# NTT123/vietTTS

Hardware: AMD Instinct MI355X
Metric: audio samples/sec whole-node, HiFi-GAN V1 mel2wave (higher is better)
Workload: dtype bf16; 1 GPU; HiFi-GAN V1 generator, 64 utterances x 1024 mel frames per GPU per step (BASELINE configs[2] shape), bf16; batch_per_gpu=64, frames=1024, parallelism=dp1 utterance-sharded, weights broadcast once, no data-path collective, microbatch=0, streams=0, schedule=engine default: micro-batches of <= 32768 frames on two HIP streams

## Files before the change

viettts_amd/csrc/engine.hip:

```cpp
#include "../../include/vtts_hifigan.h"

#include <hip/hip_runtime.h>

#include <cmath>
#include <cstdarg>
#include <cstdio>
#include <cstring>
#include <string>
#include <vector>

#include "vtts_internal.h"

using namespace vtts;

namespace {

thread_local std::string g_last_error;

}

int vtts::failf(int code, const char* fmt, ...) {
    char buf[512];
    va_list ap;
    va_start(ap, fmt);
// ... 50 lines not shown
    int64_t opt_profile = 0;
    int cur_b0 = 0;
    const int* cur_lens = nullptr;
    int cur_T = 0;
    int64_t opt_tiles = 0;
    int64_t opt_fuse = 2;
    int64_t opt_streams = 0;
    int64_t opt_graph = 1;
    struct GraphEntry {
        const void* mel = nullptr;
        void* wav = nullptr;
        void* ws = nullptr;
        int B = 0, T = 0, seen = 0;
        uint64_t epoch = 0, last_use = 0;
        hipGraph_t graph = nullptr;
        hipGraphExec_t exec = nullptr;
    };
    std::vector<GraphEntry> graphs;
    hipStream_t cap_stream = nullptr;
    uint64_t epoch = 0, use_clock = 0;
    int64_t opt_zigzag = 1;
    unsigned zrev_count = 0;
    int64_t opt_tail = 1;
    int64_t opt_chains = 1;
    hipEvent_t ev_chain[3] = {nullptr, nullptr, nullptr};
    hipStream_t side_streams[3] = {nullptr, nullptr, nullptr};
    hipEvent_t ev_fork = nullptr, ev_join[3] = {nullptr, nullptr, nullptr};
    int prof_C = 0, prof_K = 0;
    std::vector<std::pair<hipEvent_t, hipEvent_t>> prof_events;
    size_t prof_used = 0;
    double prof_flops = 0.0;
    std::string prof_name, prof_name_pair;
};

namespace {

int conv_same_pad_a(int k, int s) {
    const int pad_len = k + s - 2;
    return (s > k - 1) ? (k - 1) : (pad_len + 1) / 2;
}

void pick_dominant_class(vtts_hifigan* h, bool mfma_only) {
    double best_flops = -1.0;
    for (const Layer& l : h->layers) {
        if (&l == &h->layers[h->idx_pre] || l.kind != KIND_CONV || l.cin != l.cout || (mfma_only && !l.has_wp)) continue;
        double fl = 0.0;
// ... 423 lines not shown
    return launch_timed(h, l, 1, B, L, s, "bf16 kernel launch",
                        [&] { return ug ? launch_convt_g_bf16(l.bcls, a, s) : launch_conv_bf16(l.bcls, K, a, s); });
}

BConvArgs resblock_args_bf16(vtts_hifigan* h, const Layer& c1, const void* x, int B, int L, float slope_out, void* y, int acc_add, float div) {
    BConvArgs a;
    memset(&a, 0, sizeof(a));
    a.x = x;
    a.y = y;
    a.B = B;
    a.L = L;
    set_ragged(h, a, L);
    a.x_pitch = c1.cin;
    a.cin_real = c1.cin;
    a.slope_in = 0.1f;
    a.slope_out = slope_out;
    a.acc_add = acc_add;
    a.div = div;
    a.zrev = next_zrev(h);
    return a;
}

int run_pair_bf16(vtts_hifigan* h, const Layer& c1, const void* x, int B, int L, float slope_out, void* y, int acc_add, float div,
                  hipStream_t s, float* tail_wav = nullptr) {
    BConvArgs a = resblock_args_bf16(h, c1, x, B, L, slope_out, y, acc_add, div);
    a.wp = h->blob + c1.off_pw;
    a.bias = reinterpret_cast<const float*>(h->blob + c1.off_pb);
    a.dil = c1.dil;
    a.pad = c1.pad;
    a.tile_pref = (int)h->opt_tiles;
    if (tail_wav) {
        const Layer& post = h->layers[h->idx_post];
        a.tail_wav = tail_wav;
        a.tail_wf = reinterpret_cast<const float*>(h->blob + post.off_w);
        a.tail_bias = reinterpret_cast<const float*>(h->blob + post.off_b);
    }
    return launch_timed(h, c1, 2, B, L, s, "fused pair launch", [&] { return launch_pair_g_bf16(c1.cin, c1.k, a, s); });
}

int run_resblock_bf16(vtts_hifigan* h, const Layer* rb, const void* x, int B, int L, float slope_out, void* y, int acc_add, float div,
                      hipStream_t s) {
    BConvArgs a = resblock_args_bf16(h, rb[0], x, B, L, slope_out, y, acc_add, div);
    a.wp = h->blob + rb[0].off_rw;
    a.bias = reinterpret_cast<const float*>(h->blob + rb[0].off_rb);
    a.dils[0] = rb[0].dil;
    a.dils[1] = rb[2].dil;
    a.dils[2] = rb[4].dil;
    return launch_timed(h, rb[0], 0, B, L, s, "fused ResBlock launch", [&] { return launch_resblock_bf16(rb[0].cin, rb[0].k, a, s); });
}

Route route_bf16(const vtts_hifigan* h, const Layer* rb) {
    if (h->opt_fuse >= 2 && rb[0].has_rb && (h->opt_fuse >= 3 || resblock_bf16_preferred(rb[0].cin, rb[0].k))) return ROUTE_RESBLOCK;
    if (h->opt_fuse >= 1 && rb[0].has_pair && rb[2].has_pair && rb[4].has_pair) return ROUTE_PAIRS;
    return ROUTE_CONVS;
}

bool tail_fused_bf16(const vtts_hifigan* h) {
    if (!h->opt_tail || h->cfg.resblock == 2) return false;
    const Layer* rb = &h->layers[h->idx_res.back()];
    const Layer& post = h->layers[h->idx_post];
    return route_bf16(h, rb) == ROUTE_PAIRS && pair_tail_bf16_supported(rb[0].cin, rb[0].k, post.cin, post.cout, post.k);
}

size_t elem_bytes(const vtts_hifigan* h) { return h->dtype == VTTS_BF16 ? 2 : sizeof(float); }

size_t max_act_elems(const vtts_hifigan* h, int T) {
    size_t best = (size_t)h->cfg.upsample_initial_channel * T;
    long L = T;
    for (int i = 0; i < h->cfg.num_upsamples; ++i) {
        L *= h->cfg.upsample_rates[i];
        size_t e = (size_t)(h->cfg.upsample_initial_channel >> (i + 1)) * L;
        if (e > best) best = e;
    }
    return best;
}

int auto_streams(const vtts_hifigan* h) { return h->opt_streams > 0 ? (int)h->opt_streams : 2; }

int pass_frames(const vtts_hifigan* h) { return (h->dtype == VTTS_F32 && auto_streams(h) >= 2) ? 32768 : 65536; }

int microbatch_frames(const vtts_hifigan* h) { return auto_streams(h) >= 2 ? 32768 : 65536; }

int pick_microbatch(const vtts_hifigan* h, int B, int T) {
    if (h->opt_microbatch > 0) return (int)std::min<int64_t>(h->opt_microbatch, B);
// ... 95 lines not shown
    hipStream_t cs[4];
    int rc = fork_streams(h, nk, s, cs);
    for (int j = 0; j < nk && !rc; ++j) rc = chain(j, cs[j]);
    const int rj = join_streams(h, nk, s);
    return rc ? rc : rj;
}

struct Taps {
    const char* name = nullptr;
    float* out = nullptr;
    bool is(const char* tap, int i = -1) const {
        if (!name) return false;
        return i < 0 ? !strcmp(name, tap) : !strncmp(name, tap, 4) && atoi(name + 4) == i;
    }
};

struct MicroBatch {
    int b0, nb;
    hipStream_t s;
    PassBufs buf;
    bool par;
    float* wav;
    bool tail;
};

int tap_copy(const vtts_hifigan* h, const MicroBatch& m, const void* src, float* dst, size_t n) {
    const hipError_t e = h->dtype == VTTS_BF16 ? launch_bf16_to_f32(src, dst, n, m.s)
                                               : hipMemcpyAsync(dst, src, n * sizeof(float), hipMemcpyDeviceToDevice, m.s);
    if (e != hipSuccess) return failf(VTTS_ERR_HIP, "tap copy failed: %s", hipGetErrorString(e));
    return VTTS_OK;
}

__global__ __launch_bounds__(256) void mrf_mean_k(const float* __restrict__ y0, const float* __restrict__ y1, const float* __restrict__ y2,
                                                  float* __restrict__ out, size_t n, float div) {
    for (size_t i = (size_t)blockIdx.x * 256 + threadIdx.x; i < n; i += (size_t)gridDim.x * 256) {
        float v = y0[i] + y1[i];
        if (y2) v = v + y2[i];
        out[i] = v / div;
    }
}

float* f32(char* p) { return reinterpret_cast<float*>(p); }

int conv_pre_f32(vtts_hifigan* h, const MicroBatch& m, const float* mel, int T) {
    const int nm = h->cfg.num_mels;
    return run_layer(h, h->layers[h->idx_pre], Act{mel, (long)T * nm, 1, nm}, m.nb, T, 1.0f, nullptr, f32(m.buf.S), ACC_STORE, 1.f, 0,
// ... 76 lines not shown
    auto run_chain = [&](int j, hipStream_t cs, auto before_last) -> int {
        const Layer* rb = &h->layers[h->idx_res[i * nk + j]];
        char* tT = m.buf.T[j];
        char* tC = m.buf.C[j];
        const char* cur = m.buf.X;
        const bool last_rb = j == nk - 1;
        const float slope = last_rb ? next_slope : 1.0f;
        const int acc = j > 0 ? 1 : 0;
        const float div = last_rb ? (float)nk : 1.0f;
        int rc;
        if (c.resblock == 2) {
            if ((rc = run_layer_bf16(h, rb[0], cur, C, C, m.nb, L, 0.1f, 1.0f, cur, tC, 0, 1.f, cs))) return rc;
            if ((rc = before_last())) return rc;
            return run_layer_bf16(h, rb[1], tC, C, C, m.nb, L, 0.1f, slope, tC, m.buf.S, acc, div, cs);
        }
        switch (route_bf16(h, rb)) {
            case ROUTE_RESBLOCK:
                if ((rc = before_last())) return rc;
                return run_resblock_bf16(h, rb, cur, m.nb, L, slope, m.buf.S, acc, div, cs);
            case ROUTE_PAIRS:
                if ((rc = run_pair_bf16(h, rb[0], cur, m.nb, L, 1.0f, tT, 0, 1.f, cs))) return rc;
                if ((rc = run_pair_bf16(h, rb[2], tT, m.nb, L, 1.0f, tC, 0, 1.f, cs))) return rc;
                if ((rc = before_last())) return rc;
                return run_pair_bf16(h, rb[4], tC, m.nb, L, slope, m.buf.S, acc, div, cs, last_stage && last_rb && m.tail ? m.wav : nullptr);
            default:
                for (int z = 0; z < 2; ++z) {
                    if ((rc = run_layer_bf16(h, rb[2 * z], cur, C, C, m.nb, L, 0.1f, 0.1f, nullptr, tT, 0, 1.f, cs))) return rc;
                    if ((rc = run_layer_bf16(h, rb[2 * z + 1], tT, C, C, m.nb, L, 1.0f, 1.0f, cur, tC, 0, 1.f, cs))) return rc;
                    cur = tC;
                }
                if ((rc = run_layer_bf16(h, rb[4], cur, C, C, m.nb, L, 0.1f, 0.1f, nullptr, tT, 0, 1.f, cs))) return rc;
                if ((rc = before_last())) return rc;
                return run_layer_bf16(h, rb[5], tT, C, C, m.nb, L, 1.0f, slope, cur, m.buf.S, acc, div, cs);
        }
    };
    if (!m.par) {
        for (int j = 0; j < nk; ++j)
            if (int rc = run_chain(j, m.s, [] { return VTTS_OK; })) return rc;
        return VTTS_OK;
    }
    auto hip_rc = [&](hipError_t e, const char* what) -> int {
        return e == hipSuccess ? VTTS_OK : failf(VTTS_ERR_HIP, "%s failed: %s", what, hipGetErrorString(e));
    };
    return run_chains_parallel(h, nk, m.s, [&](int j, hipStream_t cs) -> int {
        int rc = run_chain(j, cs, [&]() -> int {
            return j > 0 ? hip_rc(hipStreamWaitEvent(cs, h->ev_chain[j - 1], 0), "hipStreamWaitEvent(chain)") : VTTS_OK;
// ... 19 lines not shown
    hipError_t e = launch_conv_post_bf16(a, m.wav, pre_act, m.s);
    if (e != hipSuccess) return failf(VTTS_ERR_HIP, "conv_post launch failed: %s", hipGetErrorString(e));
    return VTTS_OK;
}

struct Engine {
    int (*conv_pre)(vtts_hifigan*, const MicroBatch&, const float* mel, int T);
    int (*upsample)(vtts_hifigan*, const MicroBatch&, int i, int L);
    int (*mrf)(vtts_hifigan*, const MicroBatch&, int i, int L);
    int (*conv_post)(vtts_hifigan*, const MicroBatch&, int L, float* pre_act);
};
constexpr Engine ENGINE_F32{conv_pre_f32, upsample_f32, mrf_f32, conv_post_f32};
constexpr Engine ENGINE_BF16{conv_pre_bf16, upsample_bf16, mrf_bf16, conv_post_bf16};

int run_micro_batch(vtts_hifigan* h, const Engine& e, const MicroBatch& m, const float* mel, int T, const Taps& tap) {
    const vtts_hifigan_cfg& c = h->cfg;
    const Layer& pre = h->layers[h->idx_pre];
    int rc;
    if ((rc = e.conv_pre(h, m, mel + (size_t)m.b0 * T * c.num_mels, T))) return rc;
    if (tap.is("conv_pre") && (rc = tap_copy(h, m, m.buf.S, tap.out + (size_t)m.b0 * pre.cout * T, (size_t)m.nb * pre.cout * T))) return rc;
    long L = T;
    for (int i = 0; i < c.num_upsamples; ++i) {
        const Layer& up = h->layers[h->idx_ups[i]];
        if ((rc = e.upsample(h, m, i, (int)L))) return rc;
        L *= up.stride;
        const size_t CL = (size_t)up.cout * L;
        if (tap.is("ups_", i) && (rc = tap_copy(h, m, m.buf.X, tap.out + (size_t)m.b0 * CL, (size_t)m.nb * CL))) return rc;
        if ((rc = e.mrf(h, m, i, (int)L))) return rc;
        if (tap.is("mrf_", i) && (rc = tap_copy(h, m, m.buf.S, tap.out + (size_t)m.b0 * CL, (size_t)m.nb * CL))) return rc;
    }
    if (m.tail) return VTTS_OK;
    return e.conv_post(h, m, (int)L, tap.is("pre_tanh") ? tap.out + (size_t)m.b0 * h->hop * T : nullptr);
}

int forward_impl(vtts_hifigan* h, const float* mel, int B, int T, float* wav, void* ws, size_t ws_bytes, hipStream_t s0,
                 const Taps& tap) {
    if (!h->blob) return failf(VTTS_ERR_STATE, "forward() before pack()/bind_packed()");
    if (B <= 0 || T <= 0) return failf(VTTS_ERR_INVALID, "B and T must be positive (got B=%d, T=%d)", B, T);
    if (int rc = check_pass_size(h, B, T)) return rc;
    const PassPlan p = plan_pass(h, B, T);
    if (ws_bytes < p.bytes() || !ws) return failf(VTTS_ERR_NOMEM, "workspace too small: %zu < %zu bytes", ws_bytes, p.bytes());
    if ((reinterpret_cast<uintptr_t>(ws) & 255) != 0) return failf(VTTS_ERR_INVALID, "workspace must be 256-B aligned");
    {
        hipError_t e = hipSetDevice(h->device);
        if (e != hipSuccess) return failf(VTTS_ERR_HIP, "hipSetDevice(%d) failed: %s", h->device, hipGetErrorString(e));
    }
    const Engine& e = h->dtype == VTTS_BF16 ? ENGINE_BF16 : ENGINE_F32;
    const bool tail = h->dtype == VTTS_BF16 && !tap.name && tail_fused_bf16(h);
    hipStream_t streams[4];
    int rc = fork_streams(h, p.nstr, s0, streams);
    for (int b0 = 0; b0 < B && !rc; b0 += p.mb) {
        const int si = (b0 / p.mb) % p.nstr;
        const MicroBatch m{b0, std::min(p.mb, B - b0), streams[si], p.buffers(ws, si, h->cfg.num_kernels), p.par, wav + (size_t)b0 * h->hop * T, tail};
        h->cur_b0 = b0;
        rc = run_micro_batch(h, e, m, mel, T, tap);
    }
    const int rj = join_streams(h, p.nstr, s0);
    return rc ? rc : rj;
}

}

VTTS_API int vtts_abi_version(void) { return VTTS_ABI_VERSION; }

VTTS_API const char* vtts_last_error(void) { return g_last_error.c_str(); }

VTTS_API int vtts_hifigan_create(const vtts_hifigan_cfg* cfg, int device, int dtype, vtts_hifigan** out) {
    if (!cfg || !out) return failf(VTTS_ERR_INVALID, "null argument");
    *out = nullptr;
    if (dtype != VTTS_F32 && dtype != VTTS_BF16 && dtype != VTTS_BF16X3) return failf(VTTS_ERR_INVALID, "unknown dtype %d", dtype);
    if (cfg->num_upsamples < 1 || cfg->num_upsamples > VTTS_MAX_UPSAMPLES)
        return failf(VTTS_ERR_INVALID, "num_upsamples %d out of range", cfg->num_upsamples);
    if (cfg->num_kernels < 1 || cfg->num_kernels > VTTS_MAX_KERNELS)
        return failf(VTTS_ERR_INVALID, "num_kernels %d out of range", cfg->num_kernels);
    if (cfg->num_mels < 1 || cfg->upsample_initial_channel < 1)
        return failf(VTTS_ERR_INVALID, "num_mels / upsample_initial_channel must be positive");
// ... 482 lines not shown
    HIP_TRY(hipMalloc(&ybuf.p, n * 2));
    if (route == 1) {
        HIP_TRY(hipMalloc(&tbuf.p, n * 2));
        HIP_TRY(hipMalloc(&cbuf.p, n * 2));
    }
    int rc = VTTS_OK;
    if (launch_f32_to_bf16(x_dev, xbuf.p, n, st) != hipSuccess || launch_f32_to_bf16(y_dev, ybuf.p, n, st) != hipSuccess)
        rc = failf(VTTS_ERR_HIP, "conversion launch failed");
    if (!rc && route == 0) rc = run_resblock_bf16(h, rb, xbuf.p, B, L, slope_out, ybuf.p, acc_add, div, st);
    if (!rc && route == 1) {
        rc = run_pair_bf16(h, rb[0], xbuf.p, B, L, 1.0f, tbuf.p, 0, 1.f, st);
        if (!rc) rc = run_pair_bf16(h, rb[2], tbuf.p, B, L, 1.0f, cbuf.p, 0, 1.f, st);
        if (!rc) rc = run_pair_bf16(h, rb[4], cbuf.p, B, L, slope_out, ybuf.p, acc_add, div, st);
    }
    if (!rc && launch_bf16_to_f32(ybuf.p, y_dev, n, st) != hipSuccess) rc = failf(VTTS_ERR_HIP, "conversion launch failed");
    hipError_t e = hipStreamSynchronize(st);
    if (!rc && e != hipSuccess) rc = failf(VTTS_ERR_HIP, "run_resblock failed: %s", hipGetErrorString(e));
    return rc;
}

VTTS_API int vtts_hifigan_set_option(vtts_hifigan* h, const char* name, int64_t value) {
    if (!h || !name) return failf(VTTS_ERR_INVALID, "null argument");
    {
        static const char* const writable[] = {"kernels", "microbatch", "fuse", "streams", "graph", "zigzag", "chains", "tiles", "tail", "stage"};
        for (const char* w : writable) {
            int64_t cur = 0;
            if (!strcmp(name, w) && vtts_hifigan_get_option(h, name, &cur) == VTTS_OK && cur == value) return VTTS_OK;
        }
    }
    ++h->epoch;
    if (!strcmp(name, "kernels")) {
        if (value != 0 && value != 1) return failf(VTTS_ERR_INVALID, "kernels must be 0 (auto) or 1 (generic)");
        h->opt_kernels = value;
    } else if (!strcmp(name, "microbatch")) {
        if (value < 0) return failf(VTTS_ERR_INVALID, "microbatch must be >= 0");
        h->opt_microbatch = value;
    } else if (!strcmp(name, "fuse")) {
        if (value < 0 || value > 3) return failf(VTTS_ERR_INVALID, "fuse must be 0 (per convolution), 1 (pairs), 2 (bf16: pairs + whole ResBlocks where faster; fp32: pairs at C <= 64) or 3 (... wherever supported)");
        h->opt_fuse = value;
    } else if (!strcmp(name, "streams")) {
        if (value < 0 || value > 4) return failf(VTTS_ERR_INVALID, "streams must be 1..4 (0 = the engine's default)");
        h->opt_streams = value;
    } else if (!strcmp(name, "graph")) {
        if (value != 0 && value != 1) return failf(VTTS_ERR_INVALID, "graph must be 0 (always eager) or 1 (small launches replay a captured hipGraph)");
        h->opt_graph = value;
    } else if (!strcmp(name, "zigzag")) {
        if (value != 0 && value != 1) return failf(VTTS_ERR_INVALID, "zigzag must be 0 or 1");
        h->opt_zigzag = value;
    } else if (!strcmp(name, "chains")) {
        if (value < 0 || value > 2) return failf(VTTS_ERR_INVALID, "chains must be 0 (ResBlocks of a stage one after the other), 1 (side by side on small fp32 launches) or 2 (... on every single-micro-batch launch)");
        h->opt_chains = value;
    } else if (!strcmp(name, "tiles")) {
        if (value < 0 || value > 2) return failf(VTTS_ERR_INVALID, "tiles must be 0 (auto), 1 (wide) or 2 (narrow)");
        h->opt_tiles = value;
    } else if (!strcmp(name, "tail")) {
        if (value != 0 && value != 1) return failf(VTTS_ERR_INVALID, "tail must be 0 or 1");
        h->opt_tail = value;
    } else if (!strcmp(name, "stage")) {
        if (value != 0) return failf(VTTS_ERR_INVALID, "stage must be 0: the whole-stage kernel was removed (it measured slower, profiles/r06_a_stage_kernel_findings.md)");
    } else if (!strcmp(name, "profile")) {
        h->opt_profile = value ? 1 : 0;
    } else if (!strcmp(name, "hop") || !strcmp(name, "pass_frames") || !strcmp(name, "max_frames_per_pass") || !strcmp(name, "graphs_cached") ||
               !strcmp(name, "profile_C") || !strcmp(name, "profile_K")) {
        return failf(VTTS_ERR_INVALID, "option '%s' is read-only", name);
    } else {
        return failf(VTTS_ERR_INVALID, "unknown option '%s'", name);
    }
    return VTTS_OK;
}

VTTS_API int vtts_hifigan_get_option(const vtts_hifigan* h, const char* name, int64_t* value) {
    if (!h || !name || !value) return failf(VTTS_ERR_INVALID, "null argument");
    if (!strcmp(name, "kernels")) *value = h->opt_kernels;
    else if (!strcmp(name, "microbatch")) *value = h->opt_microbatch;
    else if (!strcmp(name, "profile")) *value = h->opt_profile;
    else if (!strcmp(name, "tiles")) *value = h->opt_tiles;
    else if (!strcmp(name, "streams")) *value = h->opt_streams;
    else if (!strcmp(name, "zigzag")) *value = h->opt_zigzag;
    else if (!strcmp(name, "chains")) *value = h->opt_chains;
    else if (!strcmp(name, "graph")) *value = h->opt_graph;
    else if (!strcmp(name, "tail")) *value = h->opt_tail;
    else if (!strcmp(name, "stage")) *value = 0;
    else if (!strcmp(name, "graphs_cached")) {
        *value = 0;
        for (auto& g : h->graphs) *value += g.exec ? 1 : 0;
    }
    else if (!strcmp(name, "fuse")) *value = h->opt_fuse;
    else if (!strcmp(name, "hop")) *value = h->hop;
    else if (!strcmp(name, "max_frames_per_pass")) {
        const size_t per = max_act_elems(h, 1) * elem_bytes(h);
        *value = (int64_t)((((size_t)1 << 31) + per - 1) / per);
    }
    else if (!strcmp(name, "pass_frames")) *value = pass_frames(h);
    else if (!strcmp(name, "profile_C")) *value = h->prof_C;
    else if (!strcmp(name, "profile_K")) *value = h->prof_K;
    else return failf(VTTS_ERR_INVALID, "unknown option '%s'", name);
    return VTTS_OK;
}

VTTS_API int vtts_hifigan_profile_read(vtts_hifigan* h, double* resblock_ms, int64_t* launches, double* resblock_flops,
                                       int reset) {
    if (!h) return failf(VTTS_ERR_INVALID, "null argument");
    double ms = 0.0;
    for (size_t i = 0; i < h->prof_used; ++i) {
// ... 20 lines not shown
```

viettts_amd/csrc/kernels_bf16_rbg.hip:

```cpp
#include <stdio.h>
#include <string.h>

#include <type_traits>
#include <utility>

#include "bf16_common.h"

namespace vtts {

template <class F, int... I>
__device__ __forceinline__ void static_for(std::integer_sequence<int, I...>, F&& f) {
    (f(std::integral_constant<int, I>{}), ...);
}

constexpr int XCD_MAP_MIN_TILES = 192;

template <int C_, int KS_, int N1_, int WM_, int WN_, int PA_, int MINWG_, int XC_ = C_, int BLK_ = 32>
struct GTile {
    static constexpr int C = C_, KS = KS_, N1 = N1_, WM = WM_, WN = WN_, PA = PA_, MINWG = MINWG_, BLK = BLK_;
    static constexpr int XC = XC_, NXC = C / XC;
    static constexpr int MR16 = C / WM / 16, NR16 = N1 / WN / 16, NH = NR16 / 4;
    static constexpr int KS32 = C / 32, KSX32 = XC / 32;
        static constexpr int LA16 = 3, RA16 = LA16 + 1;
    static_assert(BLK == 32 || BLK == 16, "MFMA block shape");
// ... 9 lines not shown
    static constexpr int ROWST = N1 + 2 * H2;
    static constexpr int KSTEPS = C / 16;
    static constexpr int KSX = XC / 16;
    static constexpr int NQT = KS * KSTEPS;
    static constexpr int MB = C / 32;
    static constexpr int RA = PA + 1;
    static constexpr bool UNROLL_ALL = (KSX % RA) != 0;
    static constexpr bool WREG = UNROLL_ALL && NXC == 1 && NQT * MR * 4 <= 96;
    static constexpr int XPT = (ROWSX_MAX * SPR1 + THREADS - 1) / THREADS;
    static constexpr size_t CONV_BYTES = (size_t)KS * C * C * 2;
    static_assert(C % (WM * 32) == 0 && N1 % (WN * 32) == 0, "tile/wave mismatch");
    static_assert(C % XC == 0 && (NXC == 1 || !UNROLL_ALL), "channel chunking");
    static_assert(SPR1 == 4 || SPR1 == 8 || SPR1 == 16, "X row pitch 64..256 B");
    static_assert(SPR2 == 4 || SPR2 == 8 || SPR2 == 16 || SPR2 == 32, "xt row pitch 64..512 B");
    static constexpr bool RAWRES = NXC == 1 && C == 32;
    static constexpr int RAW_BYTES = RAWRES ? tile_rows16(N1) * P1 : 0;
    static __host__ __device__ constexpr int tile_bytes(int dil) {
        const int bx = tile_rows16(N1 + 2 * H2 * dil) * P1, bt = tile_rows16(ROWST) * P2;
        return bx > bt ? bx : bt;
    }
    static constexpr bool TAIL = false;
    static constexpr int TAIL_KS = 7, TAIL_H = 3;
    static constexpr int TAIL_BYTES = 0;
    static int lds_bytes(int dil) { return tile_bytes(dil) + RAW_BYTES; }
    static_assert(tile_rows16(ROWSX_MAX) * P1 + RAW_BYTES <= 80 * 1024 || !RAWRES, "two workgroups per CU");
    static_assert(tile_rows16(ROWSX_MAX) * P1 <= 160 * 1024 && tile_rows16(ROWST) * P2 <= 160 * 1024, "LDS budget");
};

template <class B>
struct GTail : B {
    static constexpr bool TAIL = true;
    static constexpr int TAIL_BYTES = 1024;
    static int lds_bytes(int dil) { return B::tile_bytes(dil) + B::RAW_BYTES + TAIL_BYTES; }
    static_assert(B::RAWRES && B::C == 32 && B::WM == 1, "the tail lives on the C = 32 tile with the LDS-resident residual rows");
    static_assert(B::tile_bytes(B::MAXDIL) + B::RAW_BYTES + TAIL_BYTES <= 80 * 1024, "two workgroups per CU");
};

template <class T>
__global__ __launch_bounds__(T::THREADS, (T::MINWG * T::THREADS + 255) / 256) void resblock_pair_g_bf16_k(BConvArgs a) {
    constexpr int C = T::C, KS = T::KS, N1 = T::N1, WN = T::WN, PA = T::PA, RA = T::RA;
    constexpr int THREADS = T::THREADS, MR = T::MR, NR = T::NR, H2 = T::H2, NT2 = T::NT2;
    constexpr int SPR1 = T::SPR1, P1 = T::P1, SPR2 = T::SPR2, P2 = T::P2, XC = T::XC, NXC = T::NXC, KSX = T::KSX;
    constexpr int KSTEPS = T::KSTEPS, NQT = T::NQT, MB = T::MB, XPT = T::XPT;
    constexpr int BLK = T::BLK;
    constexpr bool B16 = BLK == 16;
    constexpr int MR16 = T::MR16, NR16 = T::NR16, NH = T::NH;
    static_assert(!B16 || (!T::RAWRES && !T::TAIL && !T::WREG && !T::UNROLL_ALL), "16-block tiles are the rolled-loop C >= 64 tiles");

    extern __shared__ __attribute__((aligned(16))) unsigned char lds[];
    unsigned char* xt = lds;
    [[maybe_unused]] unsigned char* const xraw = lds + (T::RAWRES ? T::tile_bytes(a.dil) : 0);

    const int tid = threadIdx.x;
    const int lane = tid & 63;
    const int wave = tid >> 6;
    const int wm = wave / WN;
    const int wn = wave % WN;
    const int l31 = lane & 31;
    const int lh = lane >> 5;
    const int l15 = lane & 15;
    const int lg = lane >> 4;
    const int b = a.zrev ? (int)(gridDim.z - 1 - blockIdx.z) : (int)blockIdx.z;
    const int Lp = a.L;
    const int L = a.lens ? min(max(a.lens[b], 0) * a.len_mul, a.L) : a.L;
    constexpr int TS = T::TAIL ? NT2 - 2 * T::TAIL_H : NT2;
    const bool xmap = (a.L + TS - 1) / TS >= XCD_MAP_MIN_TILES;
    const int nt = (L + TS - 1) / TS, r = (int)((blockIdx.x + b) & 7), lo = (r * nt) >> 3, hi = ((r + 1) * nt) >> 3;
    const int tile = xmap ? lo + (int)(blockIdx.x >> 3) : (int)blockIdx.x;
    if (xmap && tile >= hi) return;
    const int t0 = tile * TS - (T::TAIL ? T::TAIL_H : 0);
    if (t0 + (T::TAIL ? T::TAIL_H : 0) >= L) return;
    const int dil = a.dil;
    const int h1 = H2 * dil;
    const int rowsx = N1 + 2 * h1;
    const unsigned short* __restrict__ xg = static_cast<const unsigned short*>(a.x) + (size_t)b * Lp * C;
    [[maybe_unused]] const int wg_lin = blockIdx.z * gridDim.x + blockIdx.x;
    VTTS_TL_ID(a, wg_lin);
    VTTS_TL(a, wg_lin, 0);

    typedef float f32x4 __attribute__((ext_vector_type(4)));
    f32x16 acc[B16 ? 1 : MR][B16 ? 1 : NR];
    f32x16 bblk[B16 ? 1 : MR];
    f32x4 acc16[B16 ? MR16 : 1][B16 ? NR16 : 1];
    f32x4 bblk16[B16 ? MR16 : 1];
    auto load_bias = [&](const float* __restrict__ bias) {
        typedef float f32x8 __attribute__((ext_vector_type(8)));
        if constexpr (B16) {
#pragma unroll
            for (int mr = 0; mr < MR16; ++mr) bblk16[mr] = *reinterpret_cast<const f32x4*>(bias + wm * (C / T::WM) + mr * 16 + 4 * lg);
            return;
        }
#pragma unroll
        for (int mr = 0; mr < MR; ++mr) {
            const float* __restrict__ bp = bias + wm * (C / T::WM) + mr * 32 + 4 * lh;
// ... 479 lines not shown
        };
        if constexpr (T::RAWRES) {
#pragma unroll
            for (int mr = 0; mr < MR; ++mr)
#pragma unroll
                for (int p = 0; p < 2; ++p)
#pragma unroll
                    for (int nr = 0; nr < NR; ++nr) {
                        const int col = wn * (N1 / WN) + nr * 32 + l31;
                        uint4 r = *reinterpret_cast<const uint4*>(xraw + tile_off<SPR1, BLK>(col, (wm * (C / T::WM) + mr * 32 + 16 * p) / 8 + lh));
                        swap_pair(r.x, r.z);
                        swap_pair(r.y, r.w);
                        const int r0 = 8 * p;
                        acc[mr][nr][r0 + 0] = vadd_raw(bf16_lo(r.x), acc[mr][nr][r0 + 0]); acc[mr][nr][r0 + 1] = vadd_raw(bf16_hi(r.x), acc[mr][nr][r0 + 1]);
                        acc[mr][nr][r0 + 2] = vadd_raw(bf16_lo(r.y), acc[mr][nr][r0 + 2]); acc[mr][nr][r0 + 3] = vadd_raw(bf16_hi(r.y), acc[mr][nr][r0 + 3]);
                        acc[mr][nr][r0 + 4] = vadd_raw(bf16_lo(r.z), acc[mr][nr][r0 + 4]); acc[mr][nr][r0 + 5] = vadd_raw(bf16_hi(r.z), acc[mr][nr][r0 + 5]);
                        acc[mr][nr][r0 + 6] = vadd_raw(bf16_lo(r.w), acc[mr][nr][r0 + 6]); acc[mr][nr][r0 + 7] = vadd_raw(bf16_hi(r.w), acc[mr][nr][r0 + 7]);
                    }
        } else {
            add_rows(xg);
        }
        if (a.acc_add != 0) add_rows(yg);
        VTTS_TL(a, wg_lin, 12);
        if constexpr (B16) {
#pragma unroll
            for (int mr = 0; mr < MR16; ++mr) {
                const int cb = wm * (C / T::WM) + mr * 16;
#pragma unroll
                for (int j = 0; j < NR16 / 2; ++j) {
                    const int row = col16 + 32 * j;
                    const int t = t0 + row;
                    const bool ok = row < NT2 && t >= 0 && t < L;
                    float v[8];
#pragma unroll
                    for (int e = 0; e < 4; ++e) {
                        v[e] = acc16[mr][2 * j][e];
                        v[4 + e] = acc16[mr][2 * j + 1][e];
                    }
                    if (dv != 1.0f) {
#pragma unroll
                        for (int e = 0; e < 8; ++e) v[e] = v[e] * rdv;
                    }
                    if (s_out != 1.0f) {
#pragma unroll
                        for (int e = 0; e < 8; ++e) v[e] = lrelu_f(v[e], s_out);
                    }
                    unsigned p0 = pack_bf16x2(v[0], v[1]), p1 = pack_bf16x2(v[2], v[3]);
                    unsigned q0 = pack_bf16x2(v[4], v[5]), q1 = pack_bf16x2(v[6], v[7]);
                    swap_pair16(p0, q0);
                    swap_pair16(p1, q1);
                    if (ok) *reinterpret_cast<uint4*>(yg + (size_t)t * C + cb + 8 * (lg >> 1)) = make_uint4(p0, p1, q0, q1);
                }
            }
        } else {
#pragma unroll
        for (int mr = 0; mr < MR; ++mr) {
#pragma unroll
            for (int p = 0; p < 2; ++p) {
                const int cb = wm * (C / T::WM) + mr * 32 + 16 * p;
#pragma unroll
                for (int nr = 0; nr < NR; ++nr) {
                    const int row = wn * (N1 / WN) + nr * 32 + l31;
                    const int t = t0 + row;
                    const bool ok = row < NT2 && t >= 0 && t < L;
                    float v[8];
#pragma unroll
                    for (int e = 0; e < 8; ++e) v[e] = acc[mr][nr][8 * p + e];
                    if (dv != 1.0f) {
#pragma unroll
                        for (int e = 0; e < 8; ++e) v[e] = v[e] * rdv;
                    }
                    if (s_out != 1.0f) {
#pragma unroll
                        for (int e = 0; e < 8; ++e) v[e] = lrelu_f(v[e], s_out);
                    }
                    unsigned p0 = pack_bf16x2(v[0], v[1]), p1 = pack_bf16x2(v[2], v[3]);
                    unsigned q0 = pack_bf16x2(v[4], v[5]), q1 = pack_bf16x2(v[6], v[7]);
                    swap_pair(p0, q0);
                    swap_pair(p1, q1);
                    if constexpr (T::TAIL) {
                        const uint4 o = ok ? make_uint4(p0, p1, q0, q1) : make_uint4(0u, 0u, 0u, 0u);
                        if (row < NT2) *reinterpret_cast<uint4*>(xraw + tile_off<SPR1, BLK>(row, (cb >> 3) + lh)) = o;
                    } else {
                        if (ok) *reinterpret_cast<uint4*>(yg + (size_t)t * C + cb + 8 * lh) = make_uint4(p0, p1, q0, q1);
                    }
                }
            }
        }
        }
    }
    if constexpr (T::TAIL) {
        __syncthreads();
        const float* tw = reinterpret_cast<const float*>(lds + T::tile_bytes(dil) + T::RAW_BYTES);
        const float tb = a.tail_bias[0];
        for (int n = tid; n < TS; n += THREADS) {
            const int t = t0 + T::TAIL_H + n;
            if (t >= L) break;
            float accp = 0.f;
#pragma unroll
            for (int j = 0; j < T::TAIL_KS; ++j) {
#pragma unroll
                for (int c = 0; c < SPR1; ++c) {
                    const uint4 v = *reinterpret_cast<const uint4*>(xraw + tile_off<SPR1, BLK>(n + j, c));
                    const float* w = tw + j * C + c * 8;
                    accp = fmaf(w[0], bf16_lo(v.x), accp); accp = fmaf(w[1], bf16_hi(v.x), accp);
                    accp = fmaf(w[2], bf16_lo(v.y), accp); accp = fmaf(w[3], bf16_hi(v.y), accp);
                    accp = fmaf(w[4], bf16_lo(v.z), accp); accp = fmaf(w[5], bf16_hi(v.z), accp);
                    accp = fmaf(w[6], bf16_lo(v.w), accp); accp = fmaf(w[7], bf16_hi(v.w), accp);
                }
            }
            a.tail_wav[(size_t)b * Lp + t] = tanhf(accp + tb);
        }
// ... 19 lines not shown
constexpr int g_mfma_blk(int C, int KS) {
    return C == 256 ? (KS == 3 ? 16 : KS == 7 ? 32 : 16)
         : C == 128 ? (KS == 3 ? 16 : KS == 7 ? 16 : 16)
         : C == 64  ? (KS == 3 ? 32 : KS == 7 ? 16 : 16)
                    : 32;
}
template <int KS> using G128 = GTile<128, KS, KS == 3 ? VTTS_G128K3_N1 : 256, 2, 2, 3, KS == 3 ? VTTS_G128K3_WG : 2, 128, g_mfma_blk(128, KS)>;
template <int KS> using G64 = GTile<64, KS, VTTS_G64_N1, 1, 4, 3, VTTS_G64_WG, 64, g_mfma_blk(64, KS)>;
#ifndef VTTS_G32_PA
#define VTTS_G32_PA 3
#endif
template <int KS> using G32 = GTile<32, KS, VTTS_G32_N1, 1, 4, VTTS_G32_PA, VTTS_G32_WG>;
template <int KS> using G256 = GTile<256, KS, 128, 4, 1, 3, 2, 128, g_mfma_blk(256, KS)>;
template <int KS> using G256S = GTile<256, KS, 64, 4, 1, 3, 2, 128, g_mfma_blk(256, KS)>;
template <int KS> using G128S = GTile<128, KS, 128, 2, 2, 3, 2, 128, g_mfma_blk(128, KS)>;
template <int KS> using G64S = GTile<64, KS, 256, 1, 4, 3, 2, 64, g_mfma_blk(64, KS)>;
template <int KS> using G32S = GTile<32, KS, 256, 1, 4, 3, 2>;
constexpr long G_MIN_WGS = 384;
template <class T>
static hipError_t launch_g(const BConvArgs& a, hipStream_t s) {
    static DynLdsOnce once;
    if (hipError_t e = set_max_dynamic_lds(reinterpret_cast<const void*>(&resblock_pair_g_bf16_k<T>), T::lds_bytes(T::MAXDIL) + VTTS_EXP_LDS_PAD, once); e != hipSuccess) return e;
    if (a.dil < 1 || a.dil > T::MAXDIL) return hipErrorInvalidValue;
    constexpr int TS = T::TAIL ? T::NT2 - 2 * T::TAIL_H : T::NT2;
    dim3 grid((a.L + TS - 1) / TS, 1, a.B);
    if ((int)grid.x >= XCD_MAP_MIN_TILES) grid.x = (grid.x + 7) / 8 * 8;
    hipLaunchKernelGGL(resblock_pair_g_bf16_k<T>, grid, dim3(T::THREADS), T::lds_bytes(a.dil) + VTTS_EXP_LDS_PAD, s, a);
    return hipGetLastError();
}

template <template <int> class TT>
static hipError_t launch_g_ks(const BConvArgs& a, int K, hipStream_t s) {
    switch (K) {
        case 3: return launch_g<TT<3>>(a, s);
        case 7: return launch_g<TT<7>>(a, s);
        case 11: return launch_g<TT<11>>(a, s);
    }
    return hipErrorInvalidValue;
}

hipError_t launch_pair_g_bf16(int C, int K, const BConvArgs& a, hipStream_t s) {
    auto narrow = [&](int nt2) { return a.tile_pref == 2 || (a.tile_pref != 1 && (long)((a.L + nt2 - 1) / nt2) * a.B < G_MIN_WGS); };
    switch (C) {
        case 256: return narrow(G256<11>::NT2) ? launch_g_ks<G256S>(a, K, s) : launch_g_ks<G256>(a, K, s);
        case 128: return narrow(G128<11>::NT2) ? launch_g_ks<G128S>(a, K, s) : launch_g_ks<G128>(a, K, s);
        case 64: return narrow(G64<11>::NT2) ? launch_g_ks<G64S>(a, K, s) : launch_g_ks<G64>(a, K, s);
        case 32:
            if (a.tail_wav) {
                if (K != 11) return hipErrorInvalidValue;
                return narrow(G32<11>::NT2) ? launch_g<GTail<G32S<11>>>(a, s) : launch_g<GTail<G32<11>>>(a, s);
            }
            return narrow(G32<11>::NT2) ? launch_g_ks<G32S>(a, K, s) : launch_g_ks<G32>(a, K, s);
    }
    return hipErrorInvalidValue;
}

bool pair_tail_bf16_supported(int C, int K, int post_cin, int post_cout, int post_k) { return C == 32 && K == 11 && post_cin == 32 && post_cout == 1 && post_k == 7; }

BPackGeom pair_g_pack_geom(int C, int K) { return BPackGeom{C, C, C, K, C, 1}; }

int pair_g_mfma_blk(int C, int K) { return g_mfma_blk(C, K); }

void pair_g_pack(const float* Wc, int C, int K, unsigned short* out) {
    if (g_mfma_blk(C, K) == 16) pair_g_pack16(Wc, C, K, out);
    else bf16_pack(Wc, C, pair_g_pack_geom(C, K), out);
}

const char* pair_g_kernel_name(int C, int K) {
    static thread_local char buf[96];
    snprintf(buf, sizeof(buf), "resblock_pair_g_bf16_k<GTile<%d, %d,", C, K);
    return buf;
}

bool pair_bf16_supported(int C, int K, int dil) {
    return (C == 256 || C == 128 || C == 64 || C == 32) && (K == 3 || K == 7 || K == 11) && dil >= 1 && dil <= 5;
}

}
```

viettts_amd/csrc/vtts_internal.h:

```cpp
#pragma once

#include <hip/hip_runtime.h>
#include <stddef.h>
#include <stdint.h>
#include <string.h>

#include "../../include/vtts_hifigan.h"

#define VTTS_API extern "C" __attribute__((visibility("default")))

namespace vtts {

int failf(int code, const char* fmt, ...);

#define HIP_TRY(expr)                                                                                          \
    do {                                                                                                       \
        hipError_t _e = (expr);                                                                                \
        if (_e != hipSuccess)                                                                                  \
            return vtts::failf(VTTS_ERR_HIP, "%s failed: %s (%s:%d)", #expr, hipGetErrorString(_e), __FILE__, __LINE__); \
    } while (0)

inline size_t align_up(size_t v, size_t a) { return (v + a - 1) / a * a; }

inline int check_blob(const void* dev_blob, size_t bytes, size_t need) {
// ... 111 lines not shown
    const void* wp;
    const float* wf;
    const float* bias;
    const void* res;
    void* y;
    int B, L;
    const int* lens;
    int len_mul;
    int x_pitch;
    int cin_real;
    int dil, pad;
    int convt_halves;
    int dils[3];
    float slope_in;
    float slope_out;
    int acc_add;
    int tile_pref;
    float div;
    int zrev;
    unsigned long long* dbg;
    float* tail_wav;
    const float* tail_wf;
    const float* tail_bias;
};

struct BPackGeom { int cinp, ckc, coutp, ks, mt, tg; };

hipError_t launch_conv_bf16(int cls, int K, const BConvArgs& a, hipStream_t s);
BPackGeom bf16_pack_geom(int cls, int K);
const char* bf16_kernel_name(int cls, int K);
inline size_t bf16_packed_bytes(const BPackGeom& g) {
    const int ncc = g.cinp / g.ckc, nsl = (g.ks + g.tg - 1) / g.tg;
    return (size_t)(g.coutp / g.mt) * ncc * nsl * ((size_t)g.mt * g.tg * g.ckc * 2);
}
void bf16_pack(const float* Wc, int cin_real, const BPackGeom& g, unsigned short* out);
bool pair_bf16_supported(int C, int K, int dil);
bool pair_tail_bf16_supported(int C, int K, int post_cin, int post_cout, int post_k);
hipError_t launch_pair_g_bf16(int C, int K, const BConvArgs& a, hipStream_t s);
BPackGeom pair_g_pack_geom(int C, int K);
int pair_g_mfma_blk(int C, int K);
inline size_t pair_g_pack16_bytes(int C, int K) { return (size_t)K * (C / 32) * (C / 16) * 64 * 8 * sizeof(unsigned short); }
inline void pair_g_pack16(const float* Wc, int C, int K, unsigned short* out) {
    size_t o = 0;
    for (int tap = 0; tap < K; ++tap)
        for (int ks = 0; ks < C / 32; ++ks)
            for (int mblk = 0; mblk < C / 16; ++mblk)
                for (int lane = 0; lane < 64; ++lane)
                    for (int e = 0; e < 8; ++e) {
                        const int ci = 32 * ks + 8 * (lane >> 4) + e, co = 16 * mblk + (lane & 15);
                        out[o++] = f32_to_bf16_rne(Wc[((size_t)tap * C + ci) * C + co]);
                    }
}
void pair_g_pack(const float* Wc, int C, int K, unsigned short* out);
const char* pair_g_kernel_name(int C, int K);
bool resblock_bf16_supported(int C, int K, const int* dils);
bool resblock_bf16_preferred(int C, int K);
hipError_t launch_resblock_bf16(int C, int K, const BConvArgs& a, hipStream_t s);
hipError_t launch_convt_g_bf16(int cls, const BConvArgs& a, hipStream_t s);
BPackGeom convt_g_pack_geom(int cls);
hipError_t launch_conv_post_bf16(const BConvArgs& a, float* wav, float* pre_act, hipStream_t s);
// ... 27 lines not shown
```

Measured before the change: 439.5 million samples/s.

## Fuse ups_2/ups_3 transposed convs into the stage-ending fused pair kernel

Adds an epilogue to the k=11 fused resblock pair kernel (C=128 and C=64). It keeps the MRF output tile in LDS and runs the following stride-2 ConvTranspose upsample from there with MFMA, writing the upsampled activation directly and skipping the separate upsample launch. This removes a global write and re-read of the stage output plus one kernel launch per fused stage. In exchange, tiles need a one-frame halo, which means recomputed overlap and slightly smaller effective tiles, and the kernel carries more registers and LDS work. It is enabled by default through a new upfuse option (bits for ups_2 and ups_3).

```diff
diff --git a/viettts_amd/csrc/engine.hip b/viettts_amd/csrc/engine.hip
--- a/viettts_amd/csrc/engine.hip
+++ b/viettts_amd/csrc/engine.hip
@@ -96,6 +96,7 @@
     int64_t opt_zigzag = 1;
     unsigned zrev_count = 0;
     int64_t opt_tail = 1;
+    int64_t opt_upfuse = 3;
     int64_t opt_chains = 1;
     hipEvent_t ev_chain[3] = {nullptr, nullptr, nullptr};
     hipStream_t side_streams[3] = {nullptr, nullptr, nullptr};
@@ -565,8 +566,13 @@
 }
 
 int run_pair_bf16(vtts_hifigan* h, const Layer& c1, const void* x, int B, int L, float slope_out, void* y, int acc_add, float div,
-                  hipStream_t s, float* tail_wav = nullptr) {
+                  hipStream_t s, float* tail_wav = nullptr, const Layer* up = nullptr, void* up_y = nullptr) {
     BConvArgs a = resblock_args_bf16(h, c1, x, B, L, slope_out, y, acc_add, div);
+    if (up) {
+        a.up_wp = h->blob + up->off_ug;
+        a.up_bias = reinterpret_cast<const float*>(h->blob + up->off_b);
+        a.up_y = up_y;
+    }
     a.wp = h->blob + c1.off_pw;
     a.bias = reinterpret_cast<const float*>(h->blob + c1.off_pb);
     a.dil = c1.dil;
@@ -578,7 +584,7 @@
         a.tail_wf = reinterpret_cast<const float*>(h->blob + post.off_w);
         a.tail_bias = reinterpret_cast<const float*>(h->blob + post.off_b);
     }
-    return launch_timed(h, c1, 2, B, L, s, "fused pair launch", [&] { return launch_pair_g_bf16(c1.cin, c1.k, a, s); });
+    return launch_timed(h, c1, up ? 0 : 2, B, L, s, "fused pair launch", [&] { return launch_pair_g_bf16(c1.cin, c1.k, a, s); });
 }
 
 int run_resblock_bf16(vtts_hifigan* h, const Layer* rb, const void* x, int B, int L, float slope_out, void* y, int acc_add, float div,
@@ -603,6 +609,15 @@
     const Layer* rb = &h->layers[h->idx_res.back()];
     const Layer& post = h->layers[h->idx_post];
     return route_bf16(h, rb) == ROUTE_PAIRS && pair_tail_bf16_supported(rb[0].cin, rb[0].k, post.cin, post.cout, post.k);
+}
+
+bool up_fused_bf16(const vtts_hifigan* h, int i) {
+    if (i < 1 || i > 2 || i + 1 >= h->cfg.num_upsamples || !((h->opt_upfuse >> (i - 1)) & 1) || h->cfg.resblock != 1 || h->opt_fuse < 1) return false;
+    const int nk = h->cfg.num_kernels;
+    const Layer* rb = &h->layers[h->idx_res[i * nk + nk - 1]];
+    const Layer& up = h->layers[h->idx_ups[i + 1]];
+    return route_bf16(h, rb) == ROUTE_PAIRS && up.has_ug &&
+           pair_up_bf16_supported(rb[0].cin, rb[0].k, up.bcls, up.cin, up.cout, up.k, up.stride);
 }
 
 size_t elem_bytes(const vtts_hifigan* h) { return h->dtype == VTTS_BF16 ? 2 : sizeof(float); }
@@ -744,6 +759,7 @@
     bool par;
     float* wav;
     bool tail;
+    unsigned upfuse;
 };
 
 int tap_copy(const vtts_hifigan* h, const MicroBatch& m, const void* src, float* dst, size_t n) {
@@ -866,6 +882,8 @@
                 if ((rc = run_pair_bf16(h, rb[0], cur, m.nb, L, 1.0f, tT, 0, 1.f, cs))) return rc;
                 if ((rc = run_pair_bf16(h, rb[2], tT, m.nb, L, 1.0f, tC, 0, 1.f, cs))) return rc;
                 if ((rc = before_last())) return rc;
+                if (last_rb && ((m.upfuse >> i) & 1))
+                    return run_pair_bf16(h, rb[4], tC, m.nb, L, slope, m.buf.S, acc, div, cs, nullptr, &h->layers[h->idx_ups[i + 1]], m.buf.X);
                 return run_pair_bf16(h, rb[4], tC, m.nb, L, slope, m.buf.S, acc, div, cs, last_stage && last_rb && m.tail ? m.wav : nullptr);
             default:
                 for (int z = 0; z < 2; ++z) {
@@ -931,7 +949,8 @@
     long L = T;
     for (int i = 0; i < c.num_upsamples; ++i) {
         const Layer& up = h->layers[h->idx_ups[i]];
-        if ((rc = e.upsample(h, m, i, (int)L))) return rc;
+        const bool up_done = i > 0 && ((m.upfuse >> (i - 1)) & 1);
+        if (!up_done && (rc = e.upsample(h, m, i, (int)L))) return rc;
         L *= up.stride;
         const size_t CL = (size_t)up.cout * L;
         if (tap.is("ups_", i) && (rc = tap_copy(h, m, m.buf.X, tap.out + (size_t)m.b0 * CL, (size_t)m.nb * CL))) return rc;
@@ -956,11 +975,14 @@
     }
     const Engine& e = h->dtype == VTTS_BF16 ? ENGINE_BF16 : ENGINE_F32;
     const bool tail = h->dtype == VTTS_BF16 && !tap.name && tail_fused_bf16(h);
+    unsigned upfuse = 0;
+    for (int i = 1; h->dtype == VTTS_BF16 && i + 1 < h->cfg.num_upsamples; ++i)
+        if (up_fused_bf16(h, i) && !tap.is("mrf_", i)) upfuse |= 1u << i;
     hipStream_t streams[4];
     int rc = fork_streams(h, p.nstr, s0, streams);
     for (int b0 = 0; b0 < B && !rc; b0 += p.mb) {
         const int si = (b0 / p.mb) % p.nstr;
-        const MicroBatch m{b0, std::min(p.mb, B - b0), streams[si], p.buffers(ws, si, h->cfg.num_kernels), p.par, wav + (size_t)b0 * h->hop * T, tail};
+        const MicroBatch m{b0, std::min(p.mb, B - b0), streams[si], p.buffers(ws, si, h->cfg.num_kernels), p.par, wav + (size_t)b0 * h->hop * T, tail, upfuse};
         h->cur_b0 = b0;
         rc = run_micro_batch(h, e, m, mel, T, tap);
     }
@@ -1489,7 +1511,7 @@
 VTTS_API int vtts_hifigan_set_option(vtts_hifigan* h, const char* name, int64_t value) {
     if (!h || !name) return failf(VTTS_ERR_INVALID, "null argument");
     {
-        static const char* const writable[] = {"kernels", "microbatch", "fuse", "streams", "graph", "zigzag", "chains", "tiles", "tail", "stage"};
+        static const char* const writable[] = {"kernels", "microbatch", "fuse", "streams", "graph", "zigzag", "chains", "tiles", "tail", "upfuse", "stage"};
         for (const char* w : writable) {
             int64_t cur = 0;
             if (!strcmp(name, w) && vtts_hifigan_get_option(h, name, &cur) == VTTS_OK && cur == value) return VTTS_OK;
@@ -1523,6 +1545,9 @@
     } else if (!strcmp(name, "tail")) {
         if (value != 0 && value != 1) return failf(VTTS_ERR_INVALID, "tail must be 0 or 1");
         h->opt_tail = value;
+    } else if (!strcmp(name, "upfuse")) {
+        if (value < 0 || value > 3) return failf(VTTS_ERR_INVALID, "upfuse must be 0..3 (bit 0: ups_2, bit 1: ups_3 inside the pair launch that ends the stage before it)");
+        h->opt_upfuse = value;
     } else if (!strcmp(name, "stage")) {
         if (value != 0) return failf(VTTS_ERR_INVALID, "stage must be 0: the whole-stage kernel was removed (it measured slower, profiles/r06_a_stage_kernel_findings.md)");
     } else if (!strcmp(name, "profile")) {
@@ -1547,6 +1572,7 @@
     else if (!strcmp(name, "chains")) *value = h->opt_chains;
     else if (!strcmp(name, "graph")) *value = h->opt_graph;
     else if (!strcmp(name, "tail")) *value = h->opt_tail;
+    else if (!strcmp(name, "upfuse")) *value = h->opt_upfuse;
     else if (!strcmp(name, "stage")) *value = 0;
     else if (!strcmp(name, "graphs_cached")) {
         *value = 0;
diff --git a/viettts_amd/csrc/kernels_bf16_rbg.hip b/viettts_amd/csrc/kernels_bf16_rbg.hip
--- a/viettts_amd/csrc/kernels_bf16_rbg.hip
+++ b/viettts_amd/csrc/kernels_bf16_rbg.hip
@@ -55,6 +55,8 @@
     static constexpr bool TAIL = false;
     static constexpr int TAIL_KS = 7, TAIL_H = 3;
     static constexpr int TAIL_BYTES = 0;
+    static constexpr bool UP = false;
+    static constexpr int OH = 0;
     static int lds_bytes(int dil) { return tile_bytes(dil) + RAW_BYTES; }
     static_assert(tile_rows16(ROWSX_MAX) * P1 + RAW_BYTES <= 80 * 1024 || !RAWRES, "two workgroups per CU");
     static_assert(tile_rows16(ROWSX_MAX) * P1 <= 160 * 1024 && tile_rows16(ROWST) * P2 <= 160 * 1024, "LDS budget");
@@ -64,9 +66,25 @@
 struct GTail : B {
     static constexpr bool TAIL = true;
     static constexpr int TAIL_BYTES = 1024;
+    static constexpr int OH = B::TAIL_H;
     static int lds_bytes(int dil) { return B::tile_bytes(dil) + B::RAW_BYTES + TAIL_BYTES; }
     static_assert(B::RAWRES && B::C == 32 && B::WM == 1, "the tail lives on the C = 32 tile with the LDS-resident residual rows");
     static_assert(B::tile_bytes(B::MAXDIL) + B::RAW_BYTES + TAIL_BYTES <= 80 * 1024, "two workgroups per CU");
+};
+
+template <class B>
+struct GUp : B {
+    static constexpr bool UP = true;
+    static constexpr int OH = 1;
+    static constexpr int UWN = B::WM * B::WN;
+    static constexpr int UNR = B::N1 / UWN / 32;
+    static constexpr int UMR = B::C / 2 / 32;
+    static constexpr int UKS = B::C / 16;
+    static constexpr int UP_BYTES = 3 * B::C * B::C * 2;
+    static_assert(B::BLK == 16 && !B::RAWRES && !B::TAIL && B::NXC == 1 && (B::C == 128 || B::C == 64), "the stage-ending k = 11 classes (both run 16-blocks)");
+    static_assert(B::N1 % (UWN * 32) == 0 && UMR >= 1 && UKS % 2 == 0, "whole 32 x 32 blocks");
+    static_assert(B::N1 + 2 <= B::ROWST, "frames t0 - 1 .. t0 + N1 fit the xt tile");
+    static_assert(B::tile_bytes(B::MAXDIL) <= 80 * 1024, "two workgroups per CU");
 };
 
 template <class T>
@@ -96,13 +114,13 @@
     const int b = a.zrev ? (int)(gridDim.z - 1 - blockIdx.z) : (int)blockIdx.z;
     const int Lp = a.L;
     const int L = a.lens ? min(max(a.lens[b], 0) * a.len_mul, a.L) : a.L;
-    constexpr int TS = T::TAIL ? NT2 - 2 * T::TAIL_H : NT2;
+    constexpr int OH = T::OH, TS = NT2 - 2 * OH;
     const bool xmap = (a.L + TS - 1) / TS >= XCD_MAP_MIN_TILES;
     const int nt = (L + TS - 1) / TS, r = (int)((blockIdx.x + b) & 7), lo = (r * nt) >> 3, hi = ((r + 1) * nt) >> 3;
     const int tile = xmap ? lo + (int)(blockIdx.x >> 3) : (int)blockIdx.x;
     if (xmap && tile >= hi) return;
-    const int t0 = tile * TS - (T::TAIL ? T::TAIL_H : 0);
-    if (t0 + (T::TAIL ? T::TAIL_H : 0) >= L) return;
+    const int t0 = tile * TS - OH;
+    if (t0 + OH >= L) return;
     const int dil = a.dil;
     const int h1 = H2 * dil;
     const int rowsx = N1 + 2 * h1;
@@ -628,6 +646,10 @@
         }
         if (a.acc_add != 0) add_rows(yg);
         VTTS_TL(a, wg_lin, 12);
+        if constexpr (T::UP) {
+            __syncthreads();
+            VTTS_TL(a, wg_lin, 5);
+        }
         if constexpr (B16) {
 #pragma unroll
             for (int mr = 0; mr < MR16; ++mr) {
@@ -636,7 +658,7 @@
                 for (int j = 0; j < NR16 / 2; ++j) {
                     const int row = col16 + 32 * j;
                     const int t = t0 + row;
-                    const bool ok = row < NT2 && t >= 0 && t < L;
+                    const bool ok = (T::UP || row < NT2) && t >= 0 && t < L;
                     float v[8];
 #pragma unroll
                     for (int e = 0; e < 4; ++e) {
@@ -655,7 +677,12 @@
                     unsigned q0 = pack_bf16x2(v[4], v[5]), q1 = pack_bf16x2(v[6], v[7]);
                     swap_pair16(p0, q0);
                     swap_pair16(p1, q1);
-                    if (ok) *reinterpret_cast<uint4*>(yg + (size_t)t * C + cb + 8 * (lg >> 1)) = make_uint4(p0, p1, q0, q1);
+                    if constexpr (T::UP) {
+                        const uint4 o = ok ? make_uint4(p0, p1, q0, q1) : make_uint4(0u, 0u, 0u, 0u);
+                        *reinterpret_cast<uint4*>(xt + tile_off<SPR2, 32>(row, (cb >> 3) + (lg >> 1))) = o;
+                    } else {
+                        if (ok) *reinterpret_cast<uint4*>(yg + (size_t)t * C + cb + 8 * (lg >> 1)) = make_uint4(p0, p1, q0, q1);
+                    }
                 }
             }
         } else {
@@ -694,6 +721,71 @@
             }
         }
         }
+    }
+    if constexpr (T::UP) {
+        constexpr int UNR = T::UNR, UMR = T::UMR, UKS = T::UKS, UMB = C / 32, NQ = 2 * UKS, UPA = 3, URA = UPA + 1;
+        typedef unsigned u32x4_t __attribute__((ext_vector_type(4)));
+        const auto rs_u = __builtin_amdgcn_make_buffer_rsrc(const_cast<void*>(a.up_wp), 0, T::UP_BYTES, 0x00020000);
+        const unsigned u_voff = (unsigned)lane * 16;
+        const int ucol = wave * (N1 / T::UWN) + l31;
+        unsigned short* __restrict__ zg = static_cast<unsigned short*>(a.up_y) + (size_t)b * Lp * C;
+        f32x16 uacc[UMR][UNR], ub[2][UMR];
+        bf16x8 uaf[URA][UMR], ubf[2][UNR];
+#pragma unroll
+        for (int c = 0; c < 2; ++c)
+#pragma unroll
+            for (int mr = 0; mr < UMR; ++mr) {
+                typedef float f32x8 __attribute__((ext_vector_type(8)));
+                const float* __restrict__ bp = a.up_bias + c * (C / 2) + mr * 32 + 4 * lh;
+                const f32x4 q0 = *reinterpret_cast<const f32x4*>(bp), q1 = *reinterpret_cast<const f32x4*>(bp + 8);
+                const f32x4 q2 = *reinterpret_cast<const f32x4*>(bp + 16), q3 = *reinterpret_cast<const f32x4*>(bp + 24);
+                const f32x8 lo = __builtin_shufflevector(q0, q1, 0, 1, 2, 3, 4, 5, 6, 7), hi = __builtin_shufflevector(q2, q3, 0, 1, 2, 3, 4, 5, 6, 7);
+                ub[c][mr] = __builtin_shufflevector(lo, hi, 0, 1, 2, 3, 4, 5, 6, 7, 8, 9, 10, 11, 12, 13, 14, 15);
+            }
+        auto uload_a = [&](auto g_tag) {
+            constexpr int g = decltype(g_tag)::value, c = g / NQ, s = g % NQ, f = c + s / UKS, ks = s % UKS;
+            constexpr int soff = ((f * UKS + ks) * UMB + c * UMR) * 1024;
+#pragma unroll
+            for (int mr = 0; mr < UMR; ++mr) uaf[g % URA][mr] = __builtin_bit_cast(bf16x8, __builtin_amdgcn_raw_buffer_load_b128(rs_u, u_voff + mr * 1024, soff, 0));
+        };
+        auto uload_b = [&](auto g_tag) {
+            constexpr int g = decltype(g_tag)::value, c = g / NQ, s = g % NQ, f = c + s / UKS, ks = s % UKS;
+#pragma unroll
+            for (int nr = 0; nr < UNR; ++nr) ubf[g & 1][nr] = *reinterpret_cast<const bf16x8*>(xt + tile_off<SPR2, 32>(ucol + 32 * nr + f, 2 * ks + lh));
+        };
+        static_for(std::make_integer_sequence<int, UPA>{}, uload_a);
+        __syncthreads();
+        VTTS_TL(a, wg_lin, 13);
+        uload_b(std::integral_constant<int, 0>{});
+        static_for(std::make_integer_sequence<int, 2 * NQ>{}, [&](auto g_tag) {
+            constexpr int g = decltype(g_tag)::value, c = g / NQ, s = g % NQ;
+            constexpr bool more_a = g + UPA < 2 * NQ, more_b = g + 1 < 2 * NQ;
+            if constexpr (more_a) uload_a(std::integral_constant<int, g + UPA>{});
+            if constexpr (more_b) uload_b(std::integral_constant<int, g + 1>{});
+#pragma unroll
+            for (int mr = 0; mr < UMR; ++mr)
+#pragma unroll
+                for (int nr = 0; nr < UNR; ++nr)
+                    uacc[mr][nr] = __builtin_amdgcn_mfma_f32_32x32x16_bf16(uaf[g % URA][mr], ubf[g & 1][nr], s == 0 ? ub[c][mr] : uacc[mr][nr], 0, 0, 0);
+            pin_loads<UMR * UNR, more_a ? UMR : 0, more_b ? UNR : 0>();
+            if constexpr (s + 1 == NQ) {
+#pragma unroll
+                for (int mr = 0; mr < UMR; ++mr)
+#pragma unroll
+                    for (int p = 0; p < 2; ++p) {
+                        const int rb = c * (C / 2) + mr * 32 + 16 * p;
+#pragma unroll
+                        for (int nr = 0; nr < UNR; ++nr) {
+                            const int n = ucol + 32 * nr, q = t0 + OH + n;
+                            unsigned p0 = pack_bf16x2(uacc[mr][nr][8 * p + 0], uacc[mr][nr][8 * p + 1]), p1 = pack_bf16x2(uacc[mr][nr][8 * p + 2], uacc[mr][nr][8 * p + 3]);
+                            unsigned q0 = pack_bf16x2(uacc[mr][nr][8 * p + 4], uacc[mr][nr][8 * p + 5]), q1 = pack_bf16x2(uacc[mr][nr][8 * p + 6], uacc[mr][nr][8 * p + 7]);
+                            swap_pair(p0, q0);
+                            swap_pair(p1, q1);
+                            if (n < TS && q < L) *reinterpret_cast<uint4*>(zg + (size_t)q * C + rb + 8 * lh) = make_uint4(p0, p1, q0, q1);
+                        }
+                    }
+            }
+        });
     }
     if constexpr (T::TAIL) {
         __syncthreads();
@@ -759,7 +851,7 @@
     static DynLdsOnce once;
     if (hipError_t e = set_max_dynamic_lds(reinterpret_cast<const void*>(&resblock_pair_g_bf16_k<T>), T::lds_bytes(T::MAXDIL) + VTTS_EXP_LDS_PAD, once); e != hipSuccess) return e;
     if (a.dil < 1 || a.dil > T::MAXDIL) return hipErrorInvalidValue;
-    constexpr int TS = T::TAIL ? T::NT2 - 2 * T::TAIL_H : T::NT2;
+    constexpr int TS = T::NT2 - 2 * T::OH;
     dim3 grid((a.L + TS - 1) / TS, 1, a.B);
     if ((int)grid.x >= XCD_MAP_MIN_TILES) grid.x = (grid.x + 7) / 8 * 8;
     hipLaunchKernelGGL(resblock_pair_g_bf16_k<T>, grid, dim3(T::THREADS), T::lds_bytes(a.dil) + VTTS_EXP_LDS_PAD, s, a);
@@ -778,6 +870,12 @@
 
 hipError_t launch_pair_g_bf16(int C, int K, const BConvArgs& a, hipStream_t s) {
     auto narrow = [&](int nt2) { return a.tile_pref == 2 || (a.tile_pref != 1 && (long)((a.L + nt2 - 1) / nt2) * a.B < G_MIN_WGS); };
+    if (a.up_y) {
+        if (K != 11 || a.tail_wav) return hipErrorInvalidValue;
+        if (C == 128) return narrow(G128<11>::NT2) ? launch_g<GUp<G128S<11>>>(a, s) : launch_g<GUp<G128<11>>>(a, s);
+        if (C == 64) return narrow(G64<11>::NT2) ? launch_g<GUp<G64S<11>>>(a, s) : launch_g<GUp<G64<11>>>(a, s);
+        return hipErrorInvalidValue;
+    }
     switch (C) {
         case 256: return narrow(G256<11>::NT2) ? launch_g_ks<G256S>(a, K, s) : launch_g_ks<G256>(a, K, s);
         case 128: return narrow(G128<11>::NT2) ? launch_g_ks<G128S>(a, K, s) : launch_g_ks<G128>(a, K, s);
@@ -794,6 +892,10 @@
 
 bool pair_tail_bf16_supported(int C, int K, int post_cin, int post_cout, int post_k) { return C == 32 && K == 11 && post_cin == 32 && post_cout == 1 && post_k == 7; }
 
+bool pair_up_bf16_supported(int C, int K, int up_cls, int up_cin, int up_cout, int up_k, int up_stride) {
+    return K == 11 && ((C == 128 && up_cls == BCLS_UP2) || (C == 64 && up_cls == BCLS_UP3)) && up_cin == C && 2 * up_cout == C && up_k == 4 && up_stride == 2;
+}
+
 BPackGeom pair_g_pack_geom(int C, int K) { return BPackGeom{C, C, C, K, C, 1}; }
 
 int pair_g_mfma_blk(int C, int K) { return g_mfma_blk(C, K); }
diff --git a/viettts_amd/csrc/vtts_internal.h b/viettts_amd/csrc/vtts_internal.h
--- a/viettts_amd/csrc/vtts_internal.h
+++ b/viettts_amd/csrc/vtts_internal.h
@@ -157,6 +157,9 @@
     float* tail_wav;
     const float* tail_wf;
     const float* tail_bias;
+    const void* up_wp;
+    const float* up_bias;
+    void* up_y;
 };
 
 struct BPackGeom { int cinp, ckc, coutp, ks, mt, tg; };
@@ -171,6 +174,7 @@
 void bf16_pack(const float* Wc, int cin_real, const BPackGeom& g, unsigned short* out);
 bool pair_bf16_supported(int C, int K, int dil);
 bool pair_tail_bf16_supported(int C, int K, int post_cin, int post_cout, int post_k);
+bool pair_up_bf16_supported(int C, int K, int up_cls, int up_cin, int up_cout, int up_k, int up_stride);
 hipError_t launch_pair_g_bf16(int C, int K, const BConvArgs& a, hipStream_t s);
 BPackGeom pair_g_pack_geom(int C, int K);
 int pair_g_mfma_blk(int C, int K);
```

Result: faster. 444.8 million samples/s, median of 6 (+1.2%).
